# rnajena/dynamont

Hardware: AMD Instinct MI355X
Metric: signal samples resquiggled/sec (higher is better)
Workload: dtype f64

## Files before the change

dynamont_amd/_native.py:

```python
from __future__ import annotations

import ctypes as C
import os
import subprocess

HERE = os.path.dirname(os.path.abspath(__file__))
CSRC = os.path.join(HERE, "csrc")
LIB_PATH = os.environ.get("DYN_LIB_PATH") or os.path.join(HERE, "libdynamont_mi.so")
SOURCES = ["dynamont_mi.cpp", "buffers.cpp", "launch.cpp", "session.cpp", "async_engine.cpp", "pore_model.cpp", "csv_format.cpp", "csv_sink.cpp", "vbz_decode.cpp", "bam_reader.cpp", "rccl_comm.cpp", "model_format.cpp",
           "nt_kernels.hip", "pool_stats.hip", "wide_band.hip", "event_stats.hip", "rescale.hip", "kmer_summary.hip"]
HEADERS = ["engine.hpp", "engine_internal.hpp", "zstd_dl.hpp", "vbz_decode.hpp", "nt_kernels.hpp", "pore_model.hpp", "dp_math.hpp", "dp_math_strict.hpp", "dp_cell.hpp", "segment_kernels.hpp", "kmer_summary_kernels.hpp", "band_runs.hpp", "strict_exp_table.inc", os.path.join("..", "..", "include", "dynamont_mi.h")]

DYN_DEVICE_HOST_ONLY = -2
DYN_CSV_EVENT_STATS = 0x1
DYN_OK, DYN_ERR_INVALID_ARGUMENT, DYN_ERR_RUNTIME, DYN_ERR_DEVICE, DYN_ERR_OUT_OF_MEMORY = range(5)

c_double_p = C.POINTER(C.c_double)
c_float_p = C.POINTER(C.c_float)
c_u64_p = C.POINTER(C.c_uint64)
c_i32_p = C.POINTER(C.c_int32)
c_u8_p = C.POINTER(C.c_uint8)


class DynInfo(C.Structure):
    _fields_ = [("abi_version", C.c_int32), ("pore", C.c_int32), ("rna", C.c_int32), ("kmer_size", C.c_int32),
                ("alphabet_size", C.c_int32), ("device", C.c_int32), ("num_kmers", C.c_uint64),
                ("half_band", C.c_uint64), ("log_m1", C.c_double), ("log_e1", C.c_double), ("log_e2", C.c_double),
                ("max_half_band", C.c_uint64)]


class DynAlignOut(C.Structure):
    _fields_ = [("Z", c_double_p), ("status", c_i32_p), ("bad_char", C.c_void_p), ("seg_offsets", c_u64_p),
                ("n_segments", c_u64_p), ("sequence_positions", c_u64_p), ("signal_positions", c_u64_p),
                ("probabilities", c_double_p), ("states", c_u8_p), ("capacity", C.c_uint64)]


class DynEventOut(C.Structure):
    _fields_ = [("mean", c_double_p), ("stdev", c_double_p), ("median", c_double_p), ("capacity", C.c_uint64)]


class DynRescaleOut(C.Structure):
    _fields_ = [("shift", c_double_p), ("scale", c_double_p), ("iters_applied", c_i32_p), ("n", C.c_uint64)]


class DynTrainOut(C.Structure):
    _fields_ = [("Z", c_double_p), ("status", c_i32_p), ("bad_char", C.c_void_p), ("transitions", c_double_p),
                ("em_offsets", c_u64_p), ("em_count", c_u64_p), ("em_code", c_i32_p), ("em_mean", c_double_p),
                ("em_stdev", c_double_p), ("em_weight", c_double_p), ("em_sum", c_double_p),
                ("em_sumsq", c_double_p), ("trans_counts", c_double_p), ("capacity", C.c_uint64)]


class DynJobBatch(C.Structure):
    _fields_ = [("n", C.c_uint64),
                ("names", C.c_void_p), ("name_off", C.POINTER(C.c_uint64)), ("names_bytes", C.c_uint64),
                ("signal_ids", C.c_void_p), ("signal_id_off", C.POINTER(C.c_uint64)), ("signal_ids_bytes", C.c_uint64),
                ("signal_uuid", C.c_void_p), ("signal_uuid_ok", C.c_void_p),
                ("seqs", C.c_void_p), ("seq_off", C.POINTER(C.c_uint64)), ("seqs_bytes", C.c_uint64),
                ("shift", C.POINTER(C.c_double)), ("scale", C.POINTER(C.c_double)),
                ("start", C.POINTER(C.c_int64)), ("end", C.POINTER(C.c_int64)),
                ("n_files", C.c_uint64), ("files", C.c_void_p), ("file_off", C.POINTER(C.c_uint64)), ("files_bytes", C.c_uint64),
                ("file_id", C.POINTER(C.c_uint32)), ("bases", C.POINTER(C.c_uint32))]


class DynTiming(C.Structure):
    _fields_ = [("ms_total", C.c_double), ("ms_dp", C.c_double), ("ms_backward", C.c_double), ("ms_forward", C.c_double),
                ("ms_trace", C.c_double), ("wave_wait_share", C.c_double), ("wave_occupancy", C.c_double),
                ("cells", C.c_uint64), ("samples", C.c_uint64), ("reads_ok", C.c_uint64),
                ("launches", C.c_uint32), ("lp_inplace", C.c_uint32), ("pool_pages", C.c_uint32),
                ("page_rows", C.c_uint32), ("n_static", C.c_uint32), ("n_waves", C.c_uint32),
                ("reads_strict", C.c_uint32), ("reserved", C.c_uint32),
                ("ms_backward_strict", C.c_double), ("ms_forward_strict", C.c_double), ("cert_fallbacks", C.c_uint64),
                ("cert_rows", C.c_uint64), ("launch_share", C.c_double)]


class DynSessionStats(C.Structure):
    _fields_ = [("sessions", C.c_uint64), ("tickets", C.c_uint64), ("reads", C.c_uint64), ("cells", C.c_uint64), ("ms", C.c_double),
                ("wave_cycles_busy", C.c_uint64), ("wave_cycles_idle", C.c_uint64), ("wave_cycles_life", C.c_uint64),
                ("waves", C.c_uint64), ("aborted", C.c_uint64), ("republished", C.c_uint64)]


SIGNATURES = {
    "dyn_pore_from_string": (C.c_int, [C.c_char_p, C.POINTER(C.c_int), C.c_char_p, C.c_uint64]),
    "dyn_aligner_create": (C.c_int, [C.c_char_p, C.c_int, C.c_char_p, C.c_int, C.c_uint64, C.c_int,
                                     C.POINTER(C.c_void_p), C.c_char_p, C.c_uint64]),
    "dyn_aligner_destroy": (None, [C.c_void_p]),
    "dyn_release_cached_memory": (None, []),
    "dyn_aligner_set_model": (C.c_int, [C.c_void_p, c_double_p]),
    "dyn_format_model": (C.c_uint64, [C.c_char_p, C.c_int, c_double_p, c_double_p, C.c_uint64, C.c_char_p, C.c_uint64]),
    "dyn_aligner_info": (C.c_int, [C.c_void_p, C.POINTER(DynInfo)]),
    "dyn_aligner_model": (C.c_int, [C.c_void_p, c_double_p]),
    "dyn_aligner_session_stats": (C.c_int, [C.c_void_p, C.POINTER(DynSessionStats)]),
    "dyn_aligner_session_page_wait": (C.c_int, [C.c_void_p, c_u64_p]),
    "dyn_aligner_session_idle_split": (C.c_int, [C.c_void_p, C.POINTER(C.c_uint64)]),
    "dyn_aligner_set_session_mode": (C.c_int, [C.c_void_p, C.c_int, C.c_int]),
# ... 178 lines not shown
```

dynamont_amd/csrc/nt_kernels.hip:

```cpp
#include "nt_kernels.hpp"

#include <algorithm>

#include "band_runs.hpp"
#include "dp_cell.hpp"
#include "dp_math_strict.hpp"
#include "segment_kernels.hpp"

#define DYN_ONE_WAVE_PER_SIMD \
  __launch_bounds__(256 * DYN_WAVES_PER_SIMD) __attribute__((amdgpu_waves_per_eu(DYN_WAVES_PER_SIMD, DYN_WAVES_PER_SIMD)))

#define DYN_WAVES_PER_GROUP (4 * DYN_WAVES_PER_SIMD)

namespace dynk {

using dynmath::NEG_INF;
using dynmath::EmisV;
using dynmath::log_normal_pdf_vec;
using dynmath::SoftplusNode;
using dynmath::SoftplusLookup;
using dynmath::log_plus_issue;
using dynmath::log_plus_finish;
using dynmath::SP_NODES;

namespace {

typedef __attribute__((address_space(3))) uint32_t lds_u32_t;
typedef __attribute__((address_space(3))) uint64_t lds_u64_t;

__device__ __forceinline__ int pmod(int a) {
  int r = a % P;
  return r < 0 ? r + P : r;
}

__device__ __forceinline__ int pos_of(int lane, int j) { return j < 6 ? (j >> 1) * 128 + lane * 2 + (j & 1) : 384 + lane; }
__device__ __forceinline__ int row_pos(int s) { return pos_of(s / CPL, s % CPL); }

typedef double dyn_d2 __attribute__((ext_vector_type(2)));
typedef float dyn_f2 __attribute__((ext_vector_type(2)));
typedef float dyn_f4 __attribute__((ext_vector_type(4)));

template <bool NT>
__device__ __forceinline__ void store_row_f64(double* __restrict__ row, int lane, const double (&x)[CPL]) {
  static_assert(CPL == 7, "three register pairs and a single");
#pragma unroll
  for (int q = 0; q < 3; ++q) {
    dyn_d2 v;
    v.x = x[2 * q];
    v.y = x[2 * q + 1];
    dyn_d2* dst = reinterpret_cast<dyn_d2*>(row + q * 128 + lane * 2);
    if (NT) __builtin_nontemporal_store(v, dst);
    else *dst = v;
  }
  if (NT) __builtin_nontemporal_store(x[6], row + 384 + lane);
  else row[384 + lane] = x[6];
}

__device__ __forceinline__ uint64_t lanes_of_window(int c0, int len) {
  const int s0 = pmod(c0);
  const int l0 = s0 / CPL;
  const int n = (s0 + len - 1) / CPL - l0 + 1;
  if (n >= 64) return ~0ull;
  const uint64_t m = (1ull << n) - 1ull;
  return l0 ? ((m << l0) | (m >> (64 - l0))) : m;
}
__device__ __forceinline__ uint64_t uniform_u64(uint64_t v) {
  const uint32_t lo32 = (uint32_t)__builtin_amdgcn_readfirstlane((int)(uint32_t)v);
  const uint32_t hi32 = (uint32_t)__builtin_amdgcn_readfirstlane((int)(uint32_t)(v >> 32));
  return ((uint64_t)hi32 << 32) | lo32;
}
__device__ __forceinline__ uint64_t half_mask_of(uint64_t live) {
  uint64_t x = (live | (live >> 1)) & 0x5555555555555555ull;
  x = (x | (x >> 1)) & 0x3333333333333333ull;
  x = (x | (x >> 2)) & 0x0f0f0f0f0f0f0f0full;
  x = (x | (x >> 4)) & 0x00ff00ff00ff00ffull;
  x = (x | (x >> 8)) & 0x0000ffff0000ffffull;
  x = (x | (x >> 16)) & 0x00000000ffffffffull;
  return x;
}
#ifdef DYN_SKIP_OOB
constexpr bool SKIP_OOB = true;
#else
constexpr bool SKIP_OOB = false;
#endif
constexpr int OOB_SLACK = 5;

using dynband::band_mid;

__device__ __forceinline__ double readlane_f64(double v, int l) {
  int lo = __builtin_amdgcn_readlane(__double2loint(v), l);
  int hi = __builtin_amdgcn_readlane(__double2hiint(v), l);
  return __hiloint2double(hi, lo);
}

__device__ __forceinline__ double wave_ror1(double x) {
  int lo = __double2loint(x), hi = __double2hiint(x);
  const int rlo = __builtin_amdgcn_mov_dpp(lo, 0x13C, 0xf, 0xf, false);
  const int rhi = __builtin_amdgcn_mov_dpp(hi, 0x13C, 0xf, 0xf, false);
  return __hiloint2double(rhi, rlo);
}

__device__ __forceinline__ double wave_rol1(double x) {
  int lo = __double2loint(x), hi = __double2hiint(x);
  const int rlo = __builtin_amdgcn_mov_dpp(lo, 0x134, 0xf, 0xf, false);
  const int rhi = __builtin_amdgcn_mov_dpp(hi, 0x134, 0xf, 0xf, false);
  return __hiloint2double(rhi, rlo);
}

__device__ __forceinline__ void from_left(const double (&x)[CPL], double (&out)[CPL]) {
  out[0] = wave_ror1(x[CPL - 1]);
#pragma unroll
  for (int j = 1; j < CPL; ++j) out[j] = x[j - 1];
}

__device__ __forceinline__ void from_right(const double (&x)[CPL], double (&out)[CPL]) {
#pragma unroll
  for (int j = 0; j < CPL - 1; ++j) out[j] = x[j + 1];
  out[CPL - 1] = wave_rol1(x[0]);
}

__device__ __forceinline__ Emis load_emis(const Emis* __restrict__ pr, int n, int N) {
  Emis e;
  if (n >= 1 && n < N) {
    e = pr[n - 1];
  } else {
    e.mean = 0.0;
    e.inv_stdev = 1.0;
    e.neg_log_stdev = NEG_INF;
    e.stdev = 1.0;
  }
  return e;
}

struct WaveCtx {
  int lane;
  lds_u32_t* pt;
  int log_r;
};

struct RowCursor {
  int page = -1;
  uint32_t base = 0;
  __device__ __forceinline__ uint32_t at(const WaveCtx& w, int t) {
    const int pg = t >> w.log_r;
    if (pg != page) {
      page = pg;
      base = (uint32_t)__builtin_amdgcn_readfirstlane((int)w.pt[pg]) << w.log_r;
    }
    return base + ((uint32_t)t & ((1u << w.log_r) - 1u));
  }
};

__device__ __forceinline__ uint32_t pool_row(const WaveCtx& w, int t) {
  return (w.pt[t >> w.log_r] << w.log_r) + ((uint32_t)t & ((1u << w.log_r) - 1u));
}

__device__ __forceinline__ void wave_lds_sync() {
  __builtin_amdgcn_fence(__ATOMIC_ACQ_REL, "workgroup");
  __builtin_amdgcn_wave_barrier();
}
__device__ __forceinline__ void wave_lds_sync_local() {
  __builtin_amdgcn_fence(__ATOMIC_ACQ_REL, "workgroup", "local");
  __builtin_amdgcn_wave_barrier();
}

constexpr int RING_D = DYN_WAVES_PER_SIMD == 1 ? 4 : 2;
constexpr int ROW_BYTES = P * 8;
constexpr int RING_WAIT = 4 * (RING_D - 1);

#define DYN_DMA_MOD " nt"
__device__ __forceinline__ void ring_dma_row(const double* row_lane_ptr, unsigned lds_slot_addr) {
  asm volatile(
      "s_mov_b32 m0, %1\n\t"
      "s_nop 0\n\t"
      "global_load_lds_dwordx4 %0, off" DYN_DMA_MOD "\n\t"
      "global_load_lds_dwordx4 %0, off offset:1024" DYN_DMA_MOD "\n\t"
      "global_load_lds_dwordx4 %0, off offset:2048" DYN_DMA_MOD "\n\t"
      "s_mov_b32 exec_hi, 0\n\t"
      "global_load_lds_dwordx4 %0, off offset:3072" DYN_DMA_MOD "\n\t"
      "s_mov_b32 exec_hi, -1\n\t"
      ::"v"(row_lane_ptr), "s"(__builtin_amdgcn_readfirstlane(lds_slot_addr))
      : "memory");
}

__device__ __forceinline__ void ring_dma_row_masked(const double* row_lane_ptr, unsigned lds_slot_addr, uint64_t live, uint64_t half) {
  asm volatile(
      "s_mov_b32 m0, %1\n\t"
      "s_mov_b64 exec, %2\n\t"
      "global_load_lds_dwordx4 %0, off" DYN_DMA_MOD "\n\t"
      "global_load_lds_dwordx4 %0, off offset:1024" DYN_DMA_MOD "\n\t"
      "global_load_lds_dwordx4 %0, off offset:2048" DYN_DMA_MOD "\n\t"
      "s_mov_b64 exec, %3\n\t"
      "global_load_lds_dwordx4 %0, off offset:3072" DYN_DMA_MOD "\n\t"
      "s_mov_b64 exec, -1\n\t"
      ::"v"(row_lane_ptr), "s"(__builtin_amdgcn_readfirstlane(lds_slot_addr)), "s"(live), "s"(half)
      : "memory");
}

template <int N>
__device__ __forceinline__ void wait_vmcnt() {
  asm volatile("s_waitcnt vmcnt(%0)" ::"n"(N) : "memory");
}

__device__ __forceinline__ void ring_read_row(unsigned slot_addr, int lane, double (&b)[CPL]) {
  static_assert(CPL == 7, "ring_read_row is written for 7 cells per lane");
  dyn_d2 p0, p1, p2;
  double last;
  asm volatile(
      "ds_read_b128 %0, %4\n\t"
      "ds_read_b128 %1, %4 offset:1024\n\t"
      "ds_read_b128 %2, %4 offset:2048\n\t"
      "ds_read_b64 %3, %5 offset:3072\n\t"
      "s_waitcnt lgkmcnt(0)"
      : "=&v"(p0), "=&v"(p1), "=&v"(p2), "=&v"(last)
      : "v"(slot_addr + lane * 16), "v"(slot_addr + lane * 8)
      : "memory");
  b[0] = p0.x;
  b[1] = p0.y;
  b[2] = p1.x;
  b[3] = p1.y;
  b[4] = p2.x;
  b[5] = p2.y;
  b[6] = last;
}

template <bool STORE, int ARITH>
__device__ __forceinline__ double backward_sweep(const ReadDesc& rd, const WaveCtx& w,
                                                 const double* __restrict__ sig,
                                                 const Emis* __restrict__ par, double* __restrict__ ws,
                                                 double m1, double e2, const SoftplusNode* s_tab, uint32_t* fallbacks = nullptr) {
  const int lane = w.lane;
  uint32_t nfb = 0;
  const int T = (int)rd.T, N = (int)rd.N, bw = (int)rd.bw, W = 2 * bw + 1;
  const double ratio = rd.ratio;
  const double* __restrict__ sg = sig + rd.sig_off;
  const Emis* __restrict__ pr = par + rd.par_off;
  double* __restrict__ out = ws;
  RowCursor cur;

  bool bad_sample = false;
  int lo = band_mid(T - 1, ratio) - bw;
  const double inv_ratio = 1.0 / ratio;
  constexpr bool MASKED = SKIP_OOB && STORE && ARITH != ARITH_FOLDED;
  uint64_t store_mask = MASKED ? uniform_u64(lanes_of_window(lo - OOB_SLACK, W + 2 * OOB_SLACK)) : ~0ull;
  const int n_init = lo + bw;
  int n[CPL];
  double bE[CPL], bM[CPL], bE2[CPL], bM2[CPL], e[CPL];
  EmisV<CPL> p;
  double p_stdev[ARITH == ARITH_STRICT ? CPL : 1];
  double p_ylo[ARITH == ARITH_STRICT ? CPL : 1];
  auto set_p = [&](int j, const Emis& em) {
    set_emis<ARITH>(p, j, em);
    if constexpr (ARITH == ARITH_STRICT) {
      p_stdev[j] = em.stdev;
      p_ylo[j] = dynmath::recip_lo(em.stdev, em.inv_stdev);
    }
  };
  constexpr double SAMPLE_MAX = ARITH == ARITH_STRICT ? 1e300 : 1.7976931348623157e308;
  {
    const size_t rT = STORE ? (size_t)cur.at(w, T) * P : 0, rT1 = STORE ? (size_t)cur.at(w, T - 1) * P : 0;
#pragma unroll
    for (int j = 0; j < CPL; ++j) {
      const int slot = lane * CPL + j;
      n[j] = lo + pmod(slot - lo);
      set_p(j, load_emis(pr, n[j], (n[j] <= lo + W - 1) ? N : 0));
      bE[j] = (n[j] == n_init) ? 0.0 : NEG_INF;
      bM[j] = NEG_INF;
    }
    if (STORE) {
      store_row_f64<false>(out + rT1, lane, bE);
      store_row_f64<false>(out + rT, lane, bM);
    }
  }

  for (int thi = T - 2; thi >= 0; thi -= 64) {
    const int base = thi - 63;
    const int idx = base + lane;
    const double xs = (idx >= 0) ? sg[idx] : 0.0;
    bad_sample |= !(fabs(xs) <= SAMPLE_MAX);
    const int ilo = base < 0 ? -base : 0;
    emission_vec<ARITH>(readlane_f64(xs, 63), p, p_stdev, p_ylo, e);
    auto hand_over = [&](int new_lo) {
      const int leaving = lo + P - 1;
      const int top = lo + W - 1;
      const Emis fresh = load_emis(pr, new_lo, N);
      const Emis none = load_emis(pr, 0, 0);
#pragma unroll
      for (int j = 0; j < CPL; ++j) {
        if (n[j] == leaving) {
          n[j] = new_lo;
          set_p(j, fresh);
        }
        if (n[j] == top) {
          bE[j] = NEG_INF;
          set_p(j, none);
        }
      }
      lo = new_lo;
      if constexpr (MASKED) store_mask = uniform_u64(lanes_of_window(lo - OOB_SLACK, W + 2 * OOB_SLACK));
    };
    auto row = [&](int t, const double (&bE_in)[CPL], const double (&bM_in)[CPL], double (&bE_out)[CPL], double (&bM_out)[CPL]) {
      const int i = t - base;
      double Y[CPL], Yr[CPL], x1[CPL], x2[CPL];
#pragma unroll
      for (int j = 0; j < CPL; ++j) Y[j] = bM_in[j] + e[j];
#pragma unroll
      for (int j = 0; j < CPL; ++j) bM_out[j] = bE_in[j] + e[j];
      from_right(Y, Yr);
#pragma unroll
      for (int j = 0; j < CPL; ++j) x1[j] = Yr[j] + m1;
#pragma unroll
      for (int j = 0; j < CPL; ++j) x2[j] = bM_out[j] + e2;
      SoftplusLookup<CPL> L;
      log_plus_issue<CPL>(x1, x2, L, s_tab);
      {
        const double xnext = readlane_f64(xs, i > 0 ? i - 1 : 0);
        emission_vec<ARITH>(xnext, p, p_stdev, p_ylo, e);
      }
      if constexpr (ARITH == ARITH_FOLDED) dynmath::log_plus_finish3<CPL>(L, bE_out);
      else if constexpr (ARITH == ARITH_STRICT) log_plus_finish_certified(L, bE_out, strict_tab(s_tab), nfb);
      else log_plus_finish<CPL>(L, bE_out);
      const size_t rt = STORE ? (size_t)cur.at(w, t) * P : 0;
      if constexpr (STORE && ARITH == ARITH_FOLDED) {
        double ls[CPL];
#pragma unroll
        for (int j = 0; j < CPL; ++j) ls[j] = x2[j] - bE_out[j];
        store_row_f64<true>(out + rt, lane, ls);
      } else if (STORE) {
        if constexpr (MASKED) {
          if (__builtin_amdgcn_inverse_ballot_w64(store_mask)) store_row_f64<true>(out + rt, lane, bE_out);
        } else {
          store_row_f64<true>(out + rt, lane, bE_out);
        }
      }
    };
    int t = thi;
    const int tlo = base + ilo;
#pragma unroll 1
    while (t >= tlo) {
      const int new_lo = band_mid(t, ratio) - bw;
      if (new_lo != lo) hand_over(new_lo);
      const int tq = __builtin_amdgcn_readfirstlane(dynband::run_first_row(t, ratio, inv_ratio, tlo));
#pragma unroll 1
      for (; t - 1 >= tq; t -= 2) {
        row(t, bE, bM, bE2, bM2);
        row(t - 1, bE2, bM2, bE, bM);
      }
      if (t >= tq) {
        row(t, bE, bM, bE2, bM2);
#pragma unroll
        for (int j = 0; j < CPL; ++j) {
          bE[j] = bE2[j];
          bM[j] = bM2[j];
        }
        --t;
      }
    }
  }
  const bool any_bad = __any(bad_sample);
  if (ARITH == ARITH_STRICT && fallbacks) *fallbacks += nfb;
  return any_bad ? NEG_INF : readlane_f64(bE[0], 0);
}

__device__ __forceinline__ double max_f64(double a, double b) {
  double r;
  asm("v_max_f64 %0, %1, %2" : "=v"(r) : "v"(a), "v"(b));
  return r;
}

template <bool POST, bool INPLACE, bool STRICT>
__device__ __forceinline__ double forward_sweep(const ReadDesc& rd, const WaveCtx& w,
                                                const double* __restrict__ sig, const Emis* __restrict__ par,
                                                const double* __restrict__ ws_rd, float* __restrict__ lp_out,
                                                uint64_t* __restrict__ bits, double Z, double m1, double e2,
                                                const SoftplusNode* s_tab, unsigned ring_base, int strict_rows = 0,
                                                uint32_t* fallbacks = nullptr) {
  uint32_t nfb = 0;
  const int lane = w.lane;
  const int T = (int)rd.T, N = (int)rd.N, bw = (int)rd.bw, W = 2 * bw + 1;
  const double ratio = rd.ratio;
  const double* __restrict__ sg = sig + rd.sig_off;
  const Emis* __restrict__ pr = par + rd.par_off;
  const double* __restrict__ lat = ws_rd;
  float* __restrict__ lat_lp = lp_out;
  RowCursor cur_dma, cur_out;

  int lo = band_mid(1, ratio) - bw;
  const double inv_ratio = 1.0 / ratio;
  constexpr bool MASKED = SKIP_OOB && POST;
  uint64_t dma_mask = ~0ull, dma_half = 0xffffffffull, out_mask = ~0ull;
  auto set_masks = [&]() {
    if constexpr (MASKED) {
      dma_mask = uniform_u64(lanes_of_window(lo, W + OOB_SLACK));
      dma_half = half_mask_of(dma_mask);
      out_mask = uniform_u64(lanes_of_window(lo - 1, W + 1));
    }
  };
  set_masks();
  if constexpr (MASKED) {
    auto* ringp = (__attribute__((address_space(3))) double*)(size_t)ring_base;
#pragma unroll
    for (int k = 0; k < RING_D * P / 64; ++k) ringp[k * 64 + lane] = NEG_INF;
    wave_lds_sync_local();
  }
  int n[CPL];
  struct RowState {
    double fM[CPL], fE[CPL], e[CPL], vM[CPL], vE[CPL], b[CPL];
  };
  RowState sa, sb;
  EmisV<CPL> p;
  double p_stdev[STRICT ? CPL : 1];
  double p_ylo[STRICT ? CPL : 1];
  auto set_p = [&](int j, const Emis& e, auto with_stdev) {
    if constexpr (!POST) set_emis<ARITH_FOLDED>(p, j, e);
    else p.set(j, e);
    if constexpr (STRICT && decltype(with_stdev)::value) {
      p_stdev[j] = e.stdev;
      p_ylo[j] = dynmath::recip_lo(e.stdev, e.inv_stdev);
    }
  };
  auto emission = [&](bool strict_row, double x, double (&out)[CPL]) {
    if constexpr (STRICT) {
      if (strict_row) {
#ifdef DYN_QUOT5
        dynmath::log_normal_pdf_cert_vec<CPL>(x, p, p_stdev, out);
#else
        dynmath::log_normal_pdf_cert4_vec<CPL>(x, p, p_stdev, p_ylo, out);
#endif
        return;
      }
    }
    if constexpr (!POST) emission_vec<ARITH_FOLDED>(x, p, p_stdev, p_ylo, out);
    else log_normal_pdf_vec<CPL>(x, p, out);
  };
  const double x0 = sg[0];
  const size_t r1 = POST ? (size_t)cur_out.at(w, 1) * P : 0;
#pragma unroll
  for (int j = 0; j < CPL; ++j) {
    const int slot = lane * CPL + j;
    n[j] = lo + pmod(slot - lo);
    set_p(j, load_emis(pr, n[j], (n[j] <= lo + W - 1) ? N : 0), std::true_type{});
    sa.fE[j] = (n[j] == 0) ? 0.0 : NEG_INF;
    sa.fM[j] = NEG_INF;
    sa.vE[j] = sa.fE[j];
    sa.vM[j] = NEG_INF;
    sa.b[j] = POST ? lat[r1 + pos_of(lane, j)] : NEG_INF;
  }
  emission(1 <= strict_rows, x0, sa.e);
  const double* __restrict__ dma_src = ws_rd + lane * 2;
  if (POST) {
    for (int r = 2; r <= RING_D + 1; ++r) {
      if constexpr (MASKED) ring_dma_row_masked(dma_src + (size_t)cur_dma.at(w, min(r, T)) * P, ring_base + (r % RING_D) * ROW_BYTES, dma_mask, dma_half);
      else ring_dma_row(dma_src + (size_t)cur_dma.at(w, min(r, T)) * P, ring_base + (r % RING_D) * ROW_BYTES);
    }
  }

  auto hand_over = [&](auto strict_tag, int next_lo) {
    const Emis none = load_emis(pr, 0, 0);
    const Emis entering = load_emis(pr, lo + W, N);
#pragma unroll
    for (int j = 0; j < CPL; ++j) {
      const bool leaves = n[j] == lo;
      n[j] = leaves ? lo + P : n[j];
      if (leaves) set_p(j, none, strict_tag);
      if (n[j] == lo + W) set_p(j, entering, strict_tag);
    }
    lo = next_lo;
    set_masks();
  };

  auto row = [&](auto strict_tag, int t, double xn, const RowState& in, RowState& out) {
    constexpr bool STRICT_ROW = STRICT && decltype(strict_tag)::value;
    double fEl[CPL], vEl[CPL];
    if (POST) {
      wait_vmcnt<RING_WAIT>();
      ring_read_row(ring_base + ((t + 1) % RING_D) * ROW_BYTES, lane, out.b);
      if constexpr (MASKED)
        ring_dma_row_masked(dma_src + (size_t)cur_dma.at(w, min(t + 1 + RING_D, T)) * P, ring_base + ((t + 1) % RING_D) * ROW_BYTES, dma_mask, dma_half);
      else
        ring_dma_row(dma_src + (size_t)cur_dma.at(w, min(t + 1 + RING_D, T)) * P, ring_base + ((t + 1) % RING_D) * ROW_BYTES);
    }
    from_left(in.fE, fEl);
    if (POST) from_left(in.vE, vEl);
    double a1[CPL], a2[CPL];
#pragma unroll
    for (int j = 0; j < CPL; ++j) out.fM[j] = (fEl[j] + in.e[j]) + m1;
#pragma unroll
    for (int j = 0; j < CPL; ++j) a1[j] = in.fM[j] + in.e[j];
#pragma unroll
    for (int j = 0; j < CPL; ++j) a2[j] = (in.fE[j] + in.e[j]) + e2;
    if constexpr (STRICT_ROW) {
      SoftplusLookup<CPL> L;
      log_plus_issue<CPL>(a1, a2, L, s_tab);
      emission(true, xn, out.e);
      log_plus_finish_certified(L, out.fE, strict_tab(s_tab), nfb);
    } else {
      SoftplusLookup<CPL> L;
      log_plus_issue<CPL>(a1, a2, L, s_tab);
      emission(false, xn, out.e);
      if constexpr (!POST) dynmath::log_plus_finish3<CPL>(L, out.fE);
      else log_plus_finish<CPL>(L, out.fE);
    }
    if (POST) {
      double LPM[CPL], LPE[CPL], alt[CPL];
      uint64_t bj[CPL];
#pragma unroll
      for (int j = 0; j < CPL; ++j) LPM[j] = (out.fM[j] + (out.b[j] + out.e[j])) - Z;
#pragma unroll
      for (int j = 0; j < CPL; ++j) LPE[j] = (out.fE[j] + in.b[j]) - Z;
#pragma unroll
      for (int j = 0; j < CPL; ++j) out.vM[j] = vEl[j] + LPM[j];
#pragma unroll
      for (int j = 0; j < CPL; ++j) out.vE[j] = max_f64(in.vM[j], in.vE[j]) + LPE[j];
#pragma unroll
      for (int j = 0; j < CPL; ++j) alt[j] = in.vM[j] + LPE[j];
#pragma unroll
      for (int j = 0; j < CPL; ++j) bj[j] = __ballot(out.vE[j] == alt[j]);
      unsigned wlo, whi;
      static_assert(CPL == 7, "one v_writelane pair per cell register");
#define DYN_WL(J, LO, HI) "v_writelane_b32 %0, %" #LO ", " #J "\n\tv_writelane_b32 %1, %" #HI ", " #J "\n\t"
      asm("s_nop 4\n\t"
          DYN_WL(0, 2, 3) DYN_WL(1, 4, 5) DYN_WL(2, 6, 7) DYN_WL(3, 8, 9) DYN_WL(4, 10, 11) DYN_WL(5, 12, 13) DYN_WL(6, 14, 15)
          : "=&v"(wlo), "=&v"(whi)
          : "s"((unsigned)bj[0]), "s"((unsigned)(bj[0] >> 32)), "s"((unsigned)bj[1]), "s"((unsigned)(bj[1] >> 32)),
            "s"((unsigned)bj[2]), "s"((unsigned)(bj[2] >> 32)), "s"((unsigned)bj[3]), "s"((unsigned)(bj[3] >> 32)),
            "s"((unsigned)bj[4]), "s"((unsigned)(bj[4] >> 32)), "s"((unsigned)bj[5]), "s"((unsigned)(bj[5] >> 32)),
            "s"((unsigned)bj[6]), "s"((unsigned)(bj[6] >> 32)));
#undef DYN_WL
      const uint64_t mybits = ((uint64_t)whi << 32) | wlo;
      const uint32_t prow = cur_out.at(w, t);
      const size_t rt = (size_t)prow * P;
      const bool out_live = MASKED ? __builtin_amdgcn_inverse_ballot_w64(out_mask) : true;
      if (!out_live) {
      } else if (INPLACE) {
#pragma unroll
        for (int q = 0; q < 3; ++q) {
          dyn_f4 v4;
          v4.x = (float)LPM[2 * q];
          v4.y = (float)LPE[2 * q];
          v4.z = (float)LPM[2 * q + 1];
          v4.w = (float)LPE[2 * q + 1];
          __builtin_nontemporal_store(v4, reinterpret_cast<dyn_f4*>(&lat_lp[2 * (rt + q * 128 + lane * 2)]));
        }
        dyn_f2 v2;
        v2.x = (float)LPM[6];
        v2.y = (float)LPE[6];
        __builtin_nontemporal_store(v2, reinterpret_cast<dyn_f2*>(&lat_lp[2 * (rt + 384 + lane)]));
      } else {
#pragma unroll
        for (int q = 0; q < 3; ++q) {
          dyn_f2 v2;
          v2.x = (float)LPE[2 * q];
          v2.y = (float)LPE[2 * q + 1];
          __builtin_nontemporal_store(v2, reinterpret_cast<dyn_f2*>(&lat_lp[rt + q * 128 + lane * 2]));
        }
        __builtin_nontemporal_store((float)LPE[6], &lat_lp[rt + 384 + lane]);
      }
      if (lane < CPL) bits[(size_t)prow * CPL + lane] = mybits;
    }
  };

  auto block = [&](auto strict_tag, int tb) {
    const int idx = tb + lane;
    const double xs = (idx < T - 1) ? sg[idx] : 0.0;
    asm volatile("" ::"v"(xs));
    const int tend = tb + min(64, T - tb);
    int t = tb;
#pragma unroll 1
    while (t < tend) {
      const int next_lo = band_mid(t + 1, ratio) - bw;
      if (next_lo != lo) hand_over(strict_tag, next_lo);
      const int te = __builtin_amdgcn_readfirstlane(dynband::next_move_row(t + 1, ratio, inv_ratio, tend));
#pragma unroll 1
      for (; t + 1 < te; t += 2) {
        row(strict_tag, t, readlane_f64(xs, t - tb), sa, sb);
        row(strict_tag, t + 1, readlane_f64(xs, t + 1 - tb), sb, sa);
      }
      if (t < te) {
        row(strict_tag, t, readlane_f64(xs, t - tb), sa, sb);
        sa = sb;
        ++t;
      }
    }
  };
  int tb = 1;
  if constexpr (STRICT) {
    for (; tb < T && tb <= strict_rows; tb += 64) block(std::true_type{}, tb);
  }
  for (; tb < T; tb += 64) block(std::false_type{}, tb);
  const double (&fE)[CPL] = sa.fE;
  if (STRICT && fallbacks) *fallbacks += nfb;
  if (POST) wait_vmcnt<0>();
  const int nf = band_mid(T - 1, ratio);
  const int sf = pmod(nf);
  double zf = 0.0;
#pragma unroll
  for (int j = 0; j < CPL; ++j)
    if (j == sf % CPL) zf = fE[j];
  return readlane_f64(zf, sf / CPL);
}

__device__ __forceinline__ bool z_ok(const ReadDesc& rd, double Zf, double Zb) {
  const double size = (double)((uint64_t)rd.T * (uint64_t)(2 * rd.bw + 3));
  if (isinf(Zf) || isinf(Zb)) return false;
  return !(fabs(Zf - Zb) / size > 1e-8);
}

__device__ __forceinline__ bool traceback(const ReadDesc& rd, const WaveCtx& w, const float* __restrict__ lp,
                                          const uint64_t* __restrict__ bits, TraceBuffers tb, bool inplace,
                                          lds_u64_t* sb) {
  const int lane = w.lane;
  const int T = (int)rd.T, N = (int)rd.N;
  double* __restrict__ pp = tb.pp + rd.path_off;
  uint32_t* __restrict__ pathn = tb.pathn + rd.path_off;
  uint32_t* __restrict__ segrow = tb.segrow + rd.seg_off;

  int t = T - 1, n = N - 1;
  int slot = n % P;
  int stM = 0;
#ifndef DYN_EXP_TB_SERIAL
  uint64_t nb[CPL];
  uint32_t nprow = 0;
  auto fetch = [&](int base_) {
    const int row_ = base_ + lane;
    nprow = 0;
#pragma unroll
    for (int j = 0; j < CPL; ++j) nb[j] = 0;
    if (row_ >= 1) {
      nprow = pool_row(w, row_);
#pragma unroll
      for (int j = 0; j < CPL; ++j) nb[j] = bits[(size_t)nprow * CPL + j];
    }
  };
  int pend_row = 0, pend_n = 0, pend_st = -1;
  float pend_lp = 0.0f;
  auto finish = [&]() {
    if (pend_st >= 0) {
      if (inplace || pend_st == 0) pp[pend_row] = exp((double)pend_lp);
      pathn[pend_row] = (uint32_t)pend_n | (pend_st ? 0x80000000u : 0u);
      if (pend_st) segrow[pend_n - 1] = (uint32_t)pend_row;
    }
    pend_st = -1;
  };
  int sj = slot % CPL, sq = slot / CPL;
  if (t > 0 && n > 0) fetch(t - 63);
  while (t > 0 && n > 0) {
    const int base = t - 63;
    const int row = base + lane;
    const uint32_t prow = nprow;
#pragma unroll
    for (int j = 0; j < CPL; ++j) sb[lane * CPL + j] = nb[j];
    wave_lds_sync_local();
    if (base > 1) fetch(base - 64);
    int my_n = 0, my_st = -1;
    const int block_lo = base < 1 ? 1 : base;
    const uint64_t in_block = base >= 1 ? ~0ull : (~0ull << (1 - base));
    while (t >= block_lo && n > 0) {
      const int tl = t - base;
      if (stM) {
        if (__builtin_amdgcn_inverse_ballot_w64(1ull << tl)) {
          my_n = n;
          my_st = 1;
// ... 79 lines not shown
        slot = slot ? slot - 1 : P - 1;
        stM = 0;
        --t;
        continue;
      }
      const uint64_t wd = sb[lane * CPL + (slot % CPL)];
      const bool bit = (row >= block_lo) && (row <= t) && ((wd >> (slot / CPL)) & 1);
      const uint64_t m = __ballot(bit);
      const int r = m ? base + (63 - __builtin_clzll(m)) : block_lo - 1;
      const int e_lo = m ? r : block_lo;
      if (row >= e_lo && row <= t) {
        my_n = n;
        my_slot = slot;
        my_st = 0;
      }
      if (m) {
        t = r - 1;
        stM = 1;
      } else {
        t = block_lo - 1;
      }
    }
    if (my_st >= 0) {
      const size_t cell = (size_t)prow * P + row_pos(my_slot);
      if (inplace) pp[row] = exp((double)lp[2 * cell + (my_st ? 0 : 1)]);
      else if (my_st == 0) pp[row] = exp((double)lp[cell]);
      pathn[row] = (uint32_t)my_n | (my_st ? 0x80000000u : 0u);
      if (my_st) segrow[my_n - 1] = (uint32_t)row;
    }
    wave_lds_sync();
  }
#endif
  return t == 0 && n == 0;
}

__device__ __forceinline__ void mpost(const ReadDesc& rd, const WaveCtx& w, const double* __restrict__ bE,
                                      const float* __restrict__ lp, const double* __restrict__ sig,
                                      const Emis* __restrict__ par, TraceBuffers tb, double Zb, double m1) {
  const int T = (int)rd.T, N = (int)rd.N;
  const double* __restrict__ sg = sig + rd.sig_off;
  for (int n = 1 + w.lane; n < N; n += 64) {
    const int row = (int)tb.segrow[rd.seg_off + n - 1];
    const int slot = n % P, pslot = (n - 1) % P;
    double fE_prev;
    if (row == 1) {
      fE_prev = n == 1 ? 0.0 : NEG_INF;
    } else {
      const size_t pcell = (size_t)pool_row(w, row - 1) * P + row_pos(pslot);
      fE_prev = ((double)lp[pcell] - bE[pcell]) + Zb;
    }
    const Emis em = par[rd.par_off + n - 1];
    const double e_here = dynmath::log_normal_pdf(sg[row - 1], em);
    const double e_next = row + 1 < T ? dynmath::log_normal_pdf(sg[row], em) : NEG_INF;
    const double fM = (fE_prev + e_here) + m1;
    const double bM = bE[(size_t)pool_row(w, row + 1) * P + row_pos(slot)] + e_next;
    tb.pp[rd.path_off + row] = exp((fM + bM) - Zb);
  }
}

__device__ __forceinline__ double forward_train_chain(const ReadDesc& rd, const WaveCtx& w, const double* __restrict__ sig,
                                                      const double* __restrict__ ws, TrainBuffers tb, double Zb,
                                                      const SoftplusNode* s_tab, unsigned ring_base) {
  const int lane = w.lane;
  const int T = (int)rd.T, N = (int)rd.N, bw = (int)rd.bw;
  const double ratio = rd.ratio;
  const double* __restrict__ sg = sig + rd.sig_off;
  double* __restrict__ cw = tb.col_w + rd.par_off;
  double* __restrict__ cs1 = tb.col_s1 + rd.par_off;
  double* __restrict__ cs2 = tb.col_s2 + rd.par_off;
  const double* __restrict__ etab = exp128_tab(s_tab);
  RowCursor cur_dma;

  int lo = band_mid(1, ratio) - bw;
  double gE[CPL], gM[CPL];
  double aw[CPL], a1[CPL], a2[CPL];
  double awsum = 0.0;
#pragma unroll
  for (int j = 0; j < CPL; ++j) {
    const int nj = lo + pmod(lane * CPL + j - lo);
    gE[j] = (nj == 0) ? 1.0 : 0.0;
    gM[j] = 0.0;
    aw[j] = a1[j] = a2[j] = 0.0;
  }
  const double* __restrict__ dma_src = ws + lane * 2;
  for (int r = 0; r < RING_D; ++r)
    ring_dma_row(dma_src + (size_t)cur_dma.at(w, min(r, T)) * P, ring_base + (r % RING_D) * ROW_BYTES);

  const double one = dynmath::vreg_const(1.0);
  auto row = [&](int t, double x) {
    double ls[CPL], sp[CPL], st[CPL], mv[CPL], mvl[CPL];
    wait_vmcnt<RING_WAIT>();
    const unsigned slot_addr = ring_base + ((t - 1) % RING_D) * ROW_BYTES;
    ring_read_row(slot_addr, lane, ls);
    ring_dma_row(dma_src + (size_t)cur_dma.at(w, min(t - 1 + RING_D, T)) * P, slot_addr);
    dynmath::exp_table128_vec<CPL>(ls, sp, etab);
#pragma unroll
    for (int j = 0; j < CPL; ++j) sp[j] = dynmath::min_hw(sp[j], one);
#pragma unroll
    for (int j = 0; j < CPL; ++j) st[j] = gE[j] * sp[j];
#pragma unroll
    for (int j = 0; j < CPL; ++j) mv[j] = gE[j] - st[j];
    from_left(mv, mvl);
#pragma unroll
    for (int j = 0; j < CPL; ++j) gE[j] = gM[j] + st[j];
    const double x2 = x * x;
#pragma unroll
    for (int j = 0; j < CPL; ++j) {
      gM[j] = mvl[j];
      const double wgt = gE[j] + mvl[j];
      aw[j] += wgt;
      a1[j] = dynmath::fma_(wgt, x, a1[j]);
      a2[j] = dynmath::fma_(wgt, x2, a2[j]);
    }
    const int next_lo = band_mid(t + 1, ratio) - bw;
    if (__builtin_expect(next_lo != lo, 0)) {
#pragma unroll
      for (int j = 0; j < CPL; ++j) {
        const int nj = lo + pmod(lane * CPL + j - lo);
        if (nj == lo - 1 + P) {
          if (lo - 1 >= 1 && lo - 1 < N) {
            cw[lo - 2] = aw[j];
            cs1[lo - 2] = a1[j];
            cs2[lo - 2] = a2[j];
          }
          awsum += aw[j];
          aw[j] = a1[j] = a2[j] = 0.0;
        }
      }
      lo = next_lo;
    }
  };

  for (int tb0 = 1; tb0 < T; tb0 += 64) {
    const int idx = tb0 - 1 + lane;
    const double xs = sg[min(idx, T - 2)];
    asm volatile("" ::"v"(xs));
    const int iend = min(64, T - tb0);
#pragma unroll 1
    for (int i = 0; i < iend; ++i) row(tb0 + i, readlane_f64(xs, i));
  }
  wait_vmcnt<0>();
#pragma unroll
  for (int j = 0; j < CPL; ++j) {
    const int nj = lo + pmod(lane * CPL + j - lo);
    const int cidx = (nj == lo - 1 + P) ? lo - 1 : nj;
    if (cidx >= 1 && cidx < N) {
      cw[cidx - 1] = aw[j];
      cs1[cidx - 1] = a1[j];
      cs2[cidx - 1] = a2[j];
    }
    awsum += aw[j];
  }
  for (int off = 32; off >= 1; off >>= 1) awsum += __shfl_xor(awsum, off);
  if (lane == 0) {
    tb.trans[2 * rd.read] = (double)(N - 1);
    tb.trans[2 * rd.read + 1] = (double)(T - 1) - 2.0 * (double)(N - 1);
  }
  const int nf = band_mid(T - 1, ratio);
  const int sf = pmod(nf);
  double gf = 0.0;
#pragma unroll
  for (int j = 0; j < CPL; ++j)
    if (j == sf % CPL) gf = gE[j];
  gf = readlane_f64(gf, sf / CPL);
  const double S = (double)(T - 1);
  const bool ok = fabs(gf - 1.0) <= 1e-6 && fabs(awsum - S) <= 1e-6 * S;
  return ok ? Zb : NEG_INF;
}

__device__ __forceinline__ uint32_t ctl_load(const uint32_t* p) {
  return __hip_atomic_load(p, __ATOMIC_RELAXED, __HIP_MEMORY_SCOPE_AGENT);
}
__device__ __forceinline__ void ctl_store(uint32_t* p, uint32_t v) {
  __hip_atomic_store(p, v, __ATOMIC_RELAXED, __HIP_MEMORY_SCOPE_AGENT);
}

constexpr int CTL_LOCK = 0, CTL_HEAD = 1, CTL_FREE = 2, CTL_ABORT = 3, CTL_PROVISIONED = 4, CTL_WAITING = 5;
// ... 652 lines not shown
```

Measured before the change: 548.7.

## Strength-reduce per-row page lookups into run-based row pointers for DMA ring and stores

Replaces per-row page-table lookups (cur.at / cur_out.at) and modulo ring-slot arithmetic with row pointers that are re-seated only at page or fetch boundaries and otherwise advanced incrementally. Inner row loops are split so runs stop at page boundaries, and the DMA asm now takes a scalar base plus a per-lane offset instead of a per-lane 64-bit address. The aim is to cut scalar/vector address arithmetic and readfirstlane work in the latency-bound DP loop. In exchange it adds boundary bookkeeping and may shorten runs, and an off-by-one in the stop logic could corrupt fetches.

```diff
diff --git a/dynamont_amd/_native.py b/dynamont_amd/_native.py
--- a/dynamont_amd/_native.py
+++ b/dynamont_amd/_native.py
@@ -9,7 +9,7 @@
 LIB_PATH = os.environ.get("DYN_LIB_PATH") or os.path.join(HERE, "libdynamont_mi.so")
 SOURCES = ["dynamont_mi.cpp", "buffers.cpp", "launch.cpp", "session.cpp", "async_engine.cpp", "pore_model.cpp", "csv_format.cpp", "csv_sink.cpp", "vbz_decode.cpp", "bam_reader.cpp", "rccl_comm.cpp", "model_format.cpp",
            "nt_kernels.hip", "pool_stats.hip", "wide_band.hip", "event_stats.hip", "rescale.hip", "kmer_summary.hip"]
-HEADERS = ["engine.hpp", "engine_internal.hpp", "zstd_dl.hpp", "vbz_decode.hpp", "nt_kernels.hpp", "pore_model.hpp", "dp_math.hpp", "dp_math_strict.hpp", "dp_cell.hpp", "segment_kernels.hpp", "kmer_summary_kernels.hpp", "band_runs.hpp", "strict_exp_table.inc", os.path.join("..", "..", "include", "dynamont_mi.h")]
+HEADERS = ["engine.hpp", "engine_internal.hpp", "zstd_dl.hpp", "vbz_decode.hpp", "nt_kernels.hpp", "pore_model.hpp", "dp_math.hpp", "dp_math_strict.hpp", "dp_cell.hpp", "segment_kernels.hpp", "kmer_summary_kernels.hpp", "band_runs.hpp", "row_runs.hpp", "strict_exp_table.inc", os.path.join("..", "..", "include", "dynamont_mi.h")]
 
 DYN_DEVICE_HOST_ONLY = -2
 DYN_CSV_EVENT_STATS = 0x1
diff --git a/dynamont_amd/csrc/nt_kernels.hip b/dynamont_amd/csrc/nt_kernels.hip
--- a/dynamont_amd/csrc/nt_kernels.hip
+++ b/dynamont_amd/csrc/nt_kernels.hip
@@ -3,6 +3,7 @@
 #include <algorithm>
 
 #include "band_runs.hpp"
+#include "row_runs.hpp"
 #include "dp_cell.hpp"
 #include "dp_math_strict.hpp"
 #include "segment_kernels.hpp"
@@ -152,7 +153,7 @@
 };
 
 __device__ __forceinline__ uint32_t pool_row(const WaveCtx& w, int t) {
-  return (w.pt[t >> w.log_r] << w.log_r) + ((uint32_t)t & ((1u << w.log_r) - 1u));
+  return dynrows::pool_row(w.pt, t, w.log_r);
 }
 
 __device__ __forceinline__ void wave_lds_sync() {
@@ -167,33 +168,34 @@
 constexpr int RING_D = DYN_WAVES_PER_SIMD == 1 ? 4 : 2;
 constexpr int ROW_BYTES = P * 8;
 constexpr int RING_WAIT = 4 * (RING_D - 1);
+constexpr int RING_AHEAD = RING_D + 1;
 
 #define DYN_DMA_MOD " nt"
-__device__ __forceinline__ void ring_dma_row(const double* row_lane_ptr, unsigned lds_slot_addr) {
+__device__ __forceinline__ void ring_dma_row(const double* row, unsigned lane16, unsigned lds_slot_addr) {
   asm volatile(
-      "s_mov_b32 m0, %1\n\t"
+      "s_mov_b32 m0, %2\n\t"
       "s_nop 0\n\t"
-      "global_load_lds_dwordx4 %0, off" DYN_DMA_MOD "\n\t"
-      "global_load_lds_dwordx4 %0, off offset:1024" DYN_DMA_MOD "\n\t"
-      "global_load_lds_dwordx4 %0, off offset:2048" DYN_DMA_MOD "\n\t"
+      "global_load_lds_dwordx4 %0, %1" DYN_DMA_MOD "\n\t"
+      "global_load_lds_dwordx4 %0, %1 offset:1024" DYN_DMA_MOD "\n\t"
+      "global_load_lds_dwordx4 %0, %1 offset:2048" DYN_DMA_MOD "\n\t"
       "s_mov_b32 exec_hi, 0\n\t"
-      "global_load_lds_dwordx4 %0, off offset:3072" DYN_DMA_MOD "\n\t"
+      "global_load_lds_dwordx4 %0, %1 offset:3072" DYN_DMA_MOD "\n\t"
       "s_mov_b32 exec_hi, -1\n\t"
-      ::"v"(row_lane_ptr), "s"(__builtin_amdgcn_readfirstlane(lds_slot_addr))
+      ::"v"(lane16), "s"(row), "s"(lds_slot_addr)
       : "memory");
 }
 
-__device__ __forceinline__ void ring_dma_row_masked(const double* row_lane_ptr, unsigned lds_slot_addr, uint64_t live, uint64_t half) {
+__device__ __forceinline__ void ring_dma_row_masked(const double* row, unsigned lane16, unsigned lds_slot_addr, uint64_t live, uint64_t half) {
   asm volatile(
-      "s_mov_b32 m0, %1\n\t"
-      "s_mov_b64 exec, %2\n\t"
-      "global_load_lds_dwordx4 %0, off" DYN_DMA_MOD "\n\t"
-      "global_load_lds_dwordx4 %0, off offset:1024" DYN_DMA_MOD "\n\t"
-      "global_load_lds_dwordx4 %0, off offset:2048" DYN_DMA_MOD "\n\t"
+      "s_mov_b32 m0, %2\n\t"
       "s_mov_b64 exec, %3\n\t"
-      "global_load_lds_dwordx4 %0, off offset:3072" DYN_DMA_MOD "\n\t"
+      "global_load_lds_dwordx4 %0, %1" DYN_DMA_MOD "\n\t"
+      "global_load_lds_dwordx4 %0, %1 offset:1024" DYN_DMA_MOD "\n\t"
+      "global_load_lds_dwordx4 %0, %1 offset:2048" DYN_DMA_MOD "\n\t"
+      "s_mov_b64 exec, %4\n\t"
+      "global_load_lds_dwordx4 %0, %1 offset:3072" DYN_DMA_MOD "\n\t"
       "s_mov_b64 exec, -1\n\t"
-      ::"v"(row_lane_ptr), "s"(__builtin_amdgcn_readfirstlane(lds_slot_addr)), "s"(live), "s"(half)
+      ::"v"(lane16), "s"(row), "s"(lds_slot_addr), "s"(live), "s"(half)
       : "memory");
 }
 
@@ -202,7 +204,7 @@
   asm volatile("s_waitcnt vmcnt(%0)" ::"n"(N) : "memory");
 }
 
-__device__ __forceinline__ void ring_read_row(unsigned slot_addr, int lane, double (&b)[CPL]) {
+__device__ __forceinline__ void ring_read_row(unsigned a16, unsigned a8, double (&b)[CPL]) {
   static_assert(CPL == 7, "ring_read_row is written for 7 cells per lane");
   dyn_d2 p0, p1, p2;
   double last;
@@ -213,7 +215,7 @@
       "ds_read_b64 %3, %5 offset:3072\n\t"
       "s_waitcnt lgkmcnt(0)"
       : "=&v"(p0), "=&v"(p1), "=&v"(p2), "=&v"(last)
-      : "v"(slot_addr + lane * 16), "v"(slot_addr + lane * 8)
+      : "v"(a16), "v"(a8)
       : "memory");
   b[0] = p0.x;
   b[1] = p0.y;
@@ -272,6 +274,8 @@
       store_row_f64<false>(out + rT, lane, bM);
     }
   }
+  double* orow = nullptr;
+  int stop = T - 2;
 
   for (int thi = T - 2; thi >= 0; thi -= 64) {
     const int base = thi - 63;
@@ -320,19 +324,19 @@
       if constexpr (ARITH == ARITH_FOLDED) dynmath::log_plus_finish3<CPL>(L, bE_out);
       else if constexpr (ARITH == ARITH_STRICT) log_plus_finish_certified(L, bE_out, strict_tab(s_tab), nfb);
       else log_plus_finish<CPL>(L, bE_out);
-      const size_t rt = STORE ? (size_t)cur.at(w, t) * P : 0;
       if constexpr (STORE && ARITH == ARITH_FOLDED) {
         double ls[CPL];
 #pragma unroll
         for (int j = 0; j < CPL; ++j) ls[j] = x2[j] - bE_out[j];
-        store_row_f64<true>(out + rt, lane, ls);
+        store_row_f64<true>(orow, lane, ls);
       } else if (STORE) {
         if constexpr (MASKED) {
-          if (__builtin_amdgcn_inverse_ballot_w64(store_mask)) store_row_f64<true>(out + rt, lane, bE_out);
+          if (__builtin_amdgcn_inverse_ballot_w64(store_mask)) store_row_f64<true>(orow, lane, bE_out);
         } else {
-          store_row_f64<true>(out + rt, lane, bE_out);
-        }
-      }
+          store_row_f64<true>(orow, lane, bE_out);
+        }
+      }
+      if (STORE) orow -= P;
     };
     int t = thi;
     const int tlo = base + ilo;
@@ -340,7 +344,14 @@
     while (t >= tlo) {
       const int new_lo = band_mid(t, ratio) - bw;
       if (new_lo != lo) hand_over(new_lo);
-      const int tq = __builtin_amdgcn_readfirstlane(dynband::run_first_row(t, ratio, inv_ratio, tlo));
+      int tq = __builtin_amdgcn_readfirstlane(dynband::run_first_row(t, ratio, inv_ratio, tlo));
+      if (STORE) {
+        if (__builtin_expect(t == stop, 0)) {
+          orow = out + (size_t)cur.at(w, t) * P;
+          stop = dynrows::bwd_next_stop(t, w.log_r);
+        }
+        tq = max(tq, stop + 1);
+      }
 #pragma unroll 1
       for (; t - 1 >= tq; t -= 2) {
         row(t, bE, bM, bE2, bM2);
@@ -447,13 +458,30 @@
     sa.b[j] = POST ? lat[r1 + pos_of(lane, j)] : NEG_INF;
   }
   emission(1 <= strict_rows, x0, sa.e);
-  const double* __restrict__ dma_src = ws_rd + lane * 2;
+  const unsigned ring0 = (unsigned)__builtin_amdgcn_readfirstlane((int)ring_base);
+  const unsigned lane16 = lane * 16, lane8 = lane * 8;
   if (POST) {
-    for (int r = 2; r <= RING_D + 1; ++r) {
-      if constexpr (MASKED) ring_dma_row_masked(dma_src + (size_t)cur_dma.at(w, min(r, T)) * P, ring_base + (r % RING_D) * ROW_BYTES, dma_mask, dma_half);
-      else ring_dma_row(dma_src + (size_t)cur_dma.at(w, min(r, T)) * P, ring_base + (r % RING_D) * ROW_BYTES);
-    }
-  }
+    for (int r = 2; r <= RING_AHEAD; ++r) {
+      if constexpr (MASKED) ring_dma_row_masked(ws_rd + (size_t)cur_dma.at(w, min(r, T)) * P, lane16, ring0 + (r % RING_D) * ROW_BYTES, dma_mask, dma_half);
+      else ring_dma_row(ws_rd + (size_t)cur_dma.at(w, min(r, T)) * P, lane16, ring0 + (r % RING_D) * ROW_BYTES);
+    }
+  }
+  constexpr int LP_ROW = INPLACE ? 2 * P : P;
+  unsigned ring_slot = ring0 + ((1 + 1) % RING_D) * ROW_BYTES;
+  const double* frow = nullptr;
+  int fstep = 0;
+  float* lrow = nullptr;
+  uint64_t* brow = nullptr;
+  auto seat_store = [&](int t) {
+    const uint32_t prow = cur_out.at(w, t);
+    lrow = lat_lp + (size_t)prow * LP_ROW;
+    brow = bits + (size_t)prow * CPL;
+  };
+  auto seat_fetch = [&](int t) {
+    frow = ws_rd + (size_t)cur_dma.at(w, dynrows::fetch_row(t, T, RING_AHEAD)) * P;
+    fstep = dynrows::fetch_step(t, T, RING_AHEAD) * P;
+  };
+  int stop = 1;
 
   auto hand_over = [&](auto strict_tag, int next_lo) {
     const Emis none = load_emis(pr, 0, 0);
@@ -469,16 +497,16 @@
     set_masks();
   };
 
-  auto row = [&](auto strict_tag, int t, double xn, const RowState& in, RowState& out) {
+  auto row = [&](auto strict_tag, double xn, const RowState& in, RowState& out) {
     constexpr bool STRICT_ROW = STRICT && decltype(strict_tag)::value;
     double fEl[CPL], vEl[CPL];
     if (POST) {
       wait_vmcnt<RING_WAIT>();
-      ring_read_row(ring_base + ((t + 1) % RING_D) * ROW_BYTES, lane, out.b);
-      if constexpr (MASKED)
-        ring_dma_row_masked(dma_src + (size_t)cur_dma.at(w, min(t + 1 + RING_D, T)) * P, ring_base + ((t + 1) % RING_D) * ROW_BYTES, dma_mask, dma_half);
-      else
-        ring_dma_row(dma_src + (size_t)cur_dma.at(w, min(t + 1 + RING_D, T)) * P, ring_base + ((t + 1) % RING_D) * ROW_BYTES);
+      ring_read_row(ring_slot + lane16, ring_slot + lane8, out.b);
+      if constexpr (MASKED) ring_dma_row_masked(frow, lane16, ring_slot, dma_mask, dma_half);
+      else ring_dma_row(frow, lane16, ring_slot);
+      frow += fstep;
+      ring_slot = dynrows::ring_next(ring_slot, ring0, ROW_BYTES, RING_D);
     }
     from_left(in.fE, fEl);
     if (POST) from_left(in.vE, vEl);
@@ -528,8 +556,6 @@
             "s"((unsigned)bj[6]), "s"((unsigned)(bj[6] >> 32)));
 #undef DYN_WL
       const uint64_t mybits = ((uint64_t)whi << 32) | wlo;
-      const uint32_t prow = cur_out.at(w, t);
-      const size_t rt = (size_t)prow * P;
       const bool out_live = MASKED ? __builtin_amdgcn_inverse_ballot_w64(out_mask) : true;
       if (!out_live) {
       } else if (INPLACE) {
@@ -540,23 +566,25 @@
           v4.y = (float)LPE[2 * q];
           v4.z = (float)LPM[2 * q + 1];
           v4.w = (float)LPE[2 * q + 1];
-          __builtin_nontemporal_store(v4, reinterpret_cast<dyn_f4*>(&lat_lp[2 * (rt + q * 128 + lane * 2)]));
+          __builtin_nontemporal_store(v4, reinterpret_cast<dyn_f4*>(&lrow[2 * (q * 128 + lane * 2)]));
         }
         dyn_f2 v2;
         v2.x = (float)LPM[6];
         v2.y = (float)LPE[6];
-        __builtin_nontemporal_store(v2, reinterpret_cast<dyn_f2*>(&lat_lp[2 * (rt + 384 + lane)]));
+        __builtin_nontemporal_store(v2, reinterpret_cast<dyn_f2*>(&lrow[2 * (384 + lane)]));
       } else {
 #pragma unroll
         for (int q = 0; q < 3; ++q) {
           dyn_f2 v2;
           v2.x = (float)LPE[2 * q];
           v2.y = (float)LPE[2 * q + 1];
-          __builtin_nontemporal_store(v2, reinterpret_cast<dyn_f2*>(&lat_lp[rt + q * 128 + lane * 2]));
-        }
-        __builtin_nontemporal_store((float)LPE[6], &lat_lp[rt + 384 + lane]);
-      }
-      if (lane < CPL) bits[(size_t)prow * CPL + lane] = mybits;
+          __builtin_nontemporal_store(v2, reinterpret_cast<dyn_f2*>(&lrow[q * 128 + lane * 2]));
+        }
+        __builtin_nontemporal_store((float)LPE[6], &lrow[384 + lane]);
+      }
+      if (lane < CPL) brow[lane] = mybits;
+      lrow += LP_ROW;
+      brow += CPL;
     }
   };
 
@@ -570,14 +598,22 @@
     while (t < tend) {
       const int next_lo = band_mid(t + 1, ratio) - bw;
       if (next_lo != lo) hand_over(strict_tag, next_lo);
-      const int te = __builtin_amdgcn_readfirstlane(dynband::next_move_row(t + 1, ratio, inv_ratio, tend));
+      int te = __builtin_amdgcn_readfirstlane(dynband::next_move_row(t + 1, ratio, inv_ratio, tend));
+      if (POST) {
+        if (__builtin_expect(t == stop, 0)) {
+          seat_store(t);
+          seat_fetch(t);
+          stop = dynrows::fwd_next_stop(t, T, RING_AHEAD, w.log_r);
+        }
+        te = min(te, stop);
+      }
 #pragma unroll 1
       for (; t + 1 < te; t += 2) {
-        row(strict_tag, t, readlane_f64(xs, t - tb), sa, sb);
-        row(strict_tag, t + 1, readlane_f64(xs, t + 1 - tb), sb, sa);
+        row(strict_tag, readlane_f64(xs, t - tb), sa, sb);
+        row(strict_tag, readlane_f64(xs, t + 1 - tb), sb, sa);
       }
       if (t < te) {
-        row(strict_tag, t, readlane_f64(xs, t - tb), sa, sb);
+        row(strict_tag, readlane_f64(xs, t - tb), sa, sb);
         sa = sb;
         ++t;
       }
@@ -823,17 +859,18 @@
     gM[j] = 0.0;
     aw[j] = a1[j] = a2[j] = 0.0;
   }
-  const double* __restrict__ dma_src = ws + lane * 2;
+  const unsigned ring0 = (unsigned)__builtin_amdgcn_readfirstlane((int)ring_base);
+  const unsigned lane16 = lane * 16, lane8 = lane * 8;
   for (int r = 0; r < RING_D; ++r)
-    ring_dma_row(dma_src + (size_t)cur_dma.at(w, min(r, T)) * P, ring_base + (r % RING_D) * ROW_BYTES);
+    ring_dma_row(ws + (size_t)cur_dma.at(w, min(r, T)) * P, lane16, ring0 + (r % RING_D) * ROW_BYTES);
 
   const double one = dynmath::vreg_const(1.0);
   auto row = [&](int t, double x) {
     double ls[CPL], sp[CPL], st[CPL], mv[CPL], mvl[CPL];
     wait_vmcnt<RING_WAIT>();
-    const unsigned slot_addr = ring_base + ((t - 1) % RING_D) * ROW_BYTES;
-    ring_read_row(slot_addr, lane, ls);
-    ring_dma_row(dma_src + (size_t)cur_dma.at(w, min(t - 1 + RING_D, T)) * P, slot_addr);
+    const unsigned slot_addr = ring0 + ((t - 1) % RING_D) * ROW_BYTES;
+    ring_read_row(slot_addr + lane16, slot_addr + lane8, ls);
+    ring_dma_row(ws + (size_t)cur_dma.at(w, min(t - 1 + RING_D, T)) * P, lane16, slot_addr);
     dynmath::exp_table128_vec<CPL>(ls, sp, etab);
 #pragma unroll
     for (int j = 0; j < CPL; ++j) sp[j] = dynmath::min_hw(sp[j], one);
diff --git a/dynamont_amd/csrc/row_runs.hpp b/dynamont_amd/csrc/row_runs.hpp
--- /dev/null
+++ b/dynamont_amd/csrc/row_runs.hpp
@@ -0,0 +1,60 @@
+#pragma once
+
+#include <cstdint>
+
+#if defined(__HIPCC__)
+#include <hip/hip_runtime.h>
+#define DYN_RR_HD __host__ __device__ __forceinline__
+#else
+#define DYN_RR_HD inline
+#endif
+
+namespace dynrows {
+
+template <class PT>
+DYN_RR_HD uint32_t pool_row(PT pt, int t, int log_r) {
+  return ((uint32_t)pt[t >> log_r] << log_r) + ((uint32_t)t & ((1u << log_r) - 1u));
+}
+
+DYN_RR_HD int fetch_row(int t, int T, int ahead) {
+  const int d = t + ahead;
+  return d < T ? d : T;
+}
+DYN_RR_HD int fetch_step(int t, int T, int ahead) { return t + ahead < T ? 1 : 0; }
+
+DYN_RR_HD int fwd_run_end(int t, int te, int T, int ahead, int log_r) {
+  const int mask = (1 << log_r) - 1;
+  int e = te;
+  const int page_end = (t | mask) + 1;
+  if (page_end < e) e = page_end;
+  const int d = t + ahead;
+  if (d < T) {
+    const int fetch_page_end = t + (mask + 1 - (d & mask));
+    if (fetch_page_end < e) e = fetch_page_end;
+    const int clamp = T - ahead;
+    if (clamp < e) e = clamp;
+  }
+  return e;
+}
+DYN_RR_HD bool fwd_store_reseat(int t, int log_r) { return (t & ((1 << log_r) - 1)) == 0; }
+DYN_RR_HD bool fwd_fetch_reseat(int t, int T, int ahead, int log_r, int step) {
+  const int d = t + ahead;
+  return d < T ? (d & ((1 << log_r) - 1)) == 0 : step != 0;
+}
+
+DYN_RR_HD int fwd_next_stop(int t, int T, int ahead, int log_r) { return fwd_run_end(t, 0x7fffffff, T, ahead, log_r); }
+
+DYN_RR_HD int bwd_run_first(int t, int tq, int log_r) {
+  const int page_first = t & ~((1 << log_r) - 1);
+  return tq > page_first ? tq : page_first;
+}
+DYN_RR_HD bool bwd_store_reseat(int t, int log_r) { return ((t + 1) & ((1 << log_r) - 1)) == 0; }
+
+DYN_RR_HD int bwd_next_stop(int t, int log_r) { return (t & ~((1 << log_r) - 1)) - 1; }
+
+DYN_RR_HD unsigned ring_next(unsigned x, unsigned first, unsigned unit, unsigned ring_d) {
+  const unsigned nx = x + unit;
+  return nx == first + ring_d * unit ? first : nx;
+}
+
+}
```

Measured after the change: 556.0 (median of 6 runs). 1.3% higher.
